# RuanJohn/Mava

Hardware: AMD Instinct MI355X
Metric: env-steps/sec (whole node), ff_mappo RWARE tiny-4ag (higher is better)
Workload: dtype f32 via 2 x f16 split operands on the MFMA (3 products, f32 accumulate); 1 GPU; ff_mappo RWARE tiny-4ag-shaped synthetic obs, 4096 envs/GPU (update_batch_size=1 x num_envs=4096), rollout_length=128, ppo_epochs=4, num_minibatches=2, agents=4, obs=70/264, actions=5, one step = one PPO update = 524288 env-steps per GPU; parallelism=dp1

## Files before the change

### include/mava_hip.h

```cpp
#ifndef MAVA_HIP_H
#define MAVA_HIP_H

#include <stddef.h>
#include <stdint.h>

#ifdef __cplusplus
extern "C" {
#endif

typedef struct ihipStream_t* mava_stream_t;

const char* mava_last_error(void);
int mava_abi_version(void);

typedef struct mava_ctx mava_ctx;
enum {
  MAVA_CTX_MATMUL_MODE = 0,
  MAVA_CTX_CRITIC_AGGREGATION = 1,
  MAVA_CTX_GAE_VARIANT = 2,
  MAVA_CTX_POLICY_VARIANT = 3,
  MAVA_CTX_H2_LAUNCHES = 4,
  MAVA_CTX_TRAIN_VARIANT = 5,
  MAVA_CTX_W8_LAUNCHES = 6,
  MAVA_CTX_W1_SPLIT_FRESH = 7
};
int mava_ctx_create(mava_ctx** out);
int mava_ctx_destroy(mava_ctx* ctx);
int mava_ctx_set(mava_ctx* ctx, int key, long value);
int mava_ctx_get(const mava_ctx* ctx, int key, long* value);

int mava_gae_f32(const mava_ctx* ctx, const float* reward, const float* value, const uint8_t* done,
                 const float* last_val, const uint8_t* last_done, int T, int N, float gamma,
                 float lambda, float* adv, float* tgt, mava_stream_t s);

int mava_permutation_i32(long n, uint64_t seed, uint64_t counter, int32_t* out, mava_stream_t s);

int mava_clip_adam(float* p, const float* g, float* m, float* v, int32_t* count,
                   const int* seg_off, const float* seg_lr, int n_seg, float grad_scale,
                   float max_norm, int decay, int steps_per_update, int num_updates, float b1,
                   float b2, float eps, const float* loss_sums, float vf_coef, float ent_coef,
                   float* metrics_out, mava_stream_t s);

size_t mava_ppo_finish_workspace_bytes(int Pa, int Pc);
int mava_ppo_finish_f32(mava_ctx* ctx, const float* slab_a, long stride_a, const float* slab_c, long stride_c, int n_slab,
                        int Pa, int Pc, float* g, float* p, float* m, float* v, int32_t* count, float lr_a, float lr_c,
                        float grad_scale, float max_norm, int decay, int steps_per_update, int num_updates, float b1,
                        float b2, float eps, float vf_coef, float ent_coef, float* metrics_out, int critic_din,
                        void* workspace, size_t workspace_bytes, mava_stream_t s);

int mava_slab_reduce_f32(const float* slab, int n_slab, long slab_stride, int n, int accumulate,
                         float* out, mava_stream_t s);

int mava_slab_reduce2_f32(const float* slab, int n_slab, long slab_stride, int n_main,
                          float* out_main, int n_tail, float* out_tail, int accumulate,
                          mava_stream_t s);

int mava_mlp_param_count(int din, int n_out);
// ... 345 lines not shown
```

### mava_amd/_lib.py

```python
from __future__ import annotations

import ctypes as C
import os
from typing import Optional

import torch

_HERE = os.path.dirname(os.path.abspath(__file__))
LIB_PATH = os.environ.get("MAVA_LIB_PATH") or os.path.join(_HERE, "libmavahip.so")

_lib: Optional[C.CDLL] = None


class MavaHipError(RuntimeError):
    pass


vp = C.c_void_p
i32 = C.c_int
u32 = C.c_uint32
u64 = C.c_uint64
f32 = C.c_float
lng = C.c_long

# ... 92 lines not shown
    "mava_mat_gelu_bwd_f32": [vp, vp, lng, vp, vp],
    "mava_mat_shift_onehot_f32": [vp, vp, i32, i32, i32, i32, lng, i32, vp, vp],
    "mava_mat_sample_f32": [i32, i32, i32, i32, vp, vp, u64, u32, u32, i32, vp, vp, vp],
    "mava_mat_loss_f32": [i32, i32, i32, lng, vp, vp, vp, vp, vp, vp, vp, vp, vp, vp, i32, f32, f32, f32, f32, vp, vp, vp, i32, vp],
}
_RESTYPES = {"mava_last_error": C.c_char_p, "mava_rec_step_pack_bytes": C.c_long, "mava_ppo_finish_workspace_bytes": C.c_size_t}


def declared_symbols():
    return sorted(set(_SIGNATURES) | set(_RESTYPES))


def lib() -> C.CDLL:
    global _lib
    if _lib is None:
        if not os.path.exists(LIB_PATH):
            raise MavaHipError(
                f"{LIB_PATH} is missing: build it with `python -m mava_amd.build` "
                "(hipcc --offload-arch=gfx950). There is no CPU fallback."
            )
        _lib = C.CDLL(LIB_PATH)
        _lib.mava_last_error.restype = C.c_char_p
        _lib.mava_last_error.argtypes = []
        for name, args in _SIGNATURES.items():
            fn = getattr(_lib, name)
            fn.argtypes = args
            fn.restype = _RESTYPES.get(name, C.c_int)
    return _lib


class Ctx:

    MATMUL_MODE, CRITIC_AGGREGATION, GAE_VARIANT, POLICY_VARIANT, H2_LAUNCHES, TRAIN_VARIANT, W8_LAUNCHES, W1_SPLIT_FRESH = 0, 1, 2, 3, 4, 5, 6, 7

    def __init__(self, matmul_mode: str = "f32", critic_aggregation: bool = True):
        if matmul_mode not in ("f32", "f16x2"):
            raise ValueError(f"matmul_mode must be 'f16x2' or 'f32', got {matmul_mode!r}")
        h = C.c_void_p()
        check(lib().mava_ctx_create(C.byref(h)), "mava_ctx_create")
        self.handle: Optional[int] = h.value
        self.set(self.MATMUL_MODE, 1 if matmul_mode == "f16x2" else 0)
        self.set(self.CRITIC_AGGREGATION, int(bool(critic_aggregation)))

    def set(self, key: int, value: int) -> None:
        check(lib().mava_ctx_set(self.handle, key, int(value)), "mava_ctx_set")

    def get(self, key: int) -> int:
        out = C.c_long()
        check(lib().mava_ctx_get(self.handle, key, C.byref(out)), "mava_ctx_get")
        return int(out.value)

    @property
    def matmul_mode(self) -> str:
        return "f16x2" if self.get(self.MATMUL_MODE) == 1 else "f32"

    @property
    def h2_launches(self) -> int:
        return self.get(self.H2_LAUNCHES)

    def close(self) -> None:
        if getattr(self, "handle", None) is not None and _lib is not None:
            _lib.mava_ctx_destroy(self.handle)
        self.handle = None

    def __del__(self):
        try:
# ... 41 lines not shown
```

### mava_amd/csrc/api.cpp

```cpp
#include <stdarg.h>
#include <stdio.h>
#include <string.h>

#include "common.h"
#include "ctx.h"

static thread_local char g_err[512] = "";

void mava_set_error(const char* fmt, ...) {
  va_list ap;
  va_start(ap, fmt);
  vsnprintf(g_err, sizeof(g_err), fmt, ap);
  va_end(ap);
}

extern "C" const char* mava_last_error(void) { return g_err; }

extern "C" int mava_abi_version(void) { return 3; }

enum { CTX_MATMUL_MODE = 0, CTX_CRITIC_AGGREGATION = 1, CTX_GAE_VARIANT = 2, CTX_POLICY_VARIANT = 3, CTX_H2_LAUNCHES = 4, CTX_TRAIN_VARIANT = 5, CTX_W8_LAUNCHES = 6, CTX_W1_SPLIT_FRESH = 7 };

extern "C" int mava_ctx_create(mava_ctx** out) {
  MAVA_ARG_CHECK(out != nullptr, 0, "mava_ctx_create: null output pointer");
  mava_ctx* c = new mava_ctx();
  c->matmul_mode = 0;
  c->critic_aggregation = 1;
  c->gae_variant = 0;
  c->policy_variant = 0;
  c->h2_launches = 0;
  c->train_variant = 0;
  c->w8_launches = 0;
  c->w1_split[0] = c->w1_split[1] = nullptr;
  for (int i = 0; i < 2; ++i) {
    c->w1_fresh[i] = 0;
    c->w1_key_params[i] = nullptr;
    c->w1_key_din[i] = c->w1_key_steps[i] = 0;
  }
  *out = c;
  return MAVA_OK;
}

extern "C" int mava_ctx_destroy(mava_ctx* c) {
  if (c == nullptr) return MAVA_OK;
  for (int i = 0; i < 2; ++i)
    if (c->w1_split[i] != nullptr) (void)hipFree(c->w1_split[i]);
  delete c;
  return MAVA_OK;
}

extern "C" int mava_ctx_set(mava_ctx* c, int key, long value) {
  MAVA_ARG_CHECK(c != nullptr, 0, "mava_ctx_set: null context");
  switch (key) {
    case CTX_MATMUL_MODE:
      MAVA_ARG_CHECK(value == 0 || value == 1, 1, "mava_ctx_set: matmul mode %ld (0 = exact f32, 1 = f16x2)", value);
      c->matmul_mode = (int)value;
      c->w1_fresh[0] = c->w1_fresh[1] = 0;
      return MAVA_OK;
    case CTX_CRITIC_AGGREGATION: c->critic_aggregation = value ? 1 : 0; return MAVA_OK;
    case CTX_GAE_VARIANT: c->gae_variant = (int)value; return MAVA_OK;
    case CTX_POLICY_VARIANT: c->policy_variant = (int)value; return MAVA_OK;
    case CTX_H2_LAUNCHES: c->h2_launches = value; return MAVA_OK;
    case CTX_TRAIN_VARIANT: c->train_variant = (int)value; return MAVA_OK;
    case CTX_W8_LAUNCHES: c->w8_launches = value; return MAVA_OK;
    case CTX_W1_SPLIT_FRESH:
      MAVA_ARG_CHECK(value == 0, 1, "mava_ctx_set: MAVA_CTX_W1_SPLIT_FRESH can only be cleared (0) by the caller");
      c->w1_fresh[0] = c->w1_fresh[1] = 0;
      return MAVA_OK;
    default: mava_set_error("mava_ctx_set: unknown key %d", key); return MAVA_EARG(2);
  }
}

extern "C" int mava_ctx_get(const mava_ctx* c, int key, long* value) {
  MAVA_ARG_CHECK(c != nullptr && value != nullptr, 0, "mava_ctx_get: null argument");
  switch (key) {
    case CTX_MATMUL_MODE: *value = c->matmul_mode; return MAVA_OK;
    case CTX_CRITIC_AGGREGATION: *value = c->critic_aggregation; return MAVA_OK;
    case CTX_GAE_VARIANT: *value = c->gae_variant; return MAVA_OK;
    case CTX_POLICY_VARIANT: *value = c->policy_variant; return MAVA_OK;
    case CTX_H2_LAUNCHES: *value = c->h2_launches; return MAVA_OK;
    case CTX_TRAIN_VARIANT: *value = c->train_variant; return MAVA_OK;
    case CTX_W8_LAUNCHES: *value = c->w8_launches; return MAVA_OK;
    case CTX_W1_SPLIT_FRESH: *value = c->w1_fresh[1]; return MAVA_OK;
    default: mava_set_error("mava_ctx_get: unknown key %d", key); return MAVA_EARG(2);
  }
}
```

### mava_amd/csrc/ctx.h

```cpp
#pragma once
#include "common.h"

struct mava_ctx {
  int matmul_mode;
  int critic_aggregation;
  int gae_variant;
  int policy_variant;
  int train_variant;
  long h2_launches;
  long w8_launches;
  void* w1_split[2];
  int w1_fresh[2];
  const float* w1_key_params[2];
  int w1_key_din[2];
  int w1_key_steps[2];
};

static inline int mava_ctx_matmul_mode(const mava_ctx* c) { return c ? c->matmul_mode : 0; }
static inline int mava_ctx_critic_aggregation(const mava_ctx* c) { return c ? c->critic_aggregation : 1; }
static inline int mava_ctx_gae_variant(const mava_ctx* c) { return c ? c->gae_variant : 0; }
static inline int mava_ctx_policy_variant(const mava_ctx* c) { return c ? c->policy_variant : 0; }
```

### mava_amd/csrc/ppo_train_h2.hip

```cpp
#include "h2_core.h"
#include "ppo_train_task.h"
#include "ctx.h"

#ifndef MAVA_GW_DEPTH
#define MAVA_GW_DEPTH 0
#endif
#define GW_DEPTH MAVA_GW_DEPTH
#ifndef MAVA_GW_DEPTH_WIDE
#define MAVA_GW_DEPTH_WIDE 0
#endif

namespace {

using namespace h2;

constexpr int STATS_BLOCKS = 128;

#ifdef MAVA_STAMPS
#define STAMP_DECL unsigned long long st_prev = __builtin_readcyclecounter(), st_acc[16] = {0, 0, 0, 0, 0, 0, 0, 0, 0, 0, 0, 0, 0, 0, 0, 0};
#define STAMP(i)                                                    \
  do {                                                              \
    __builtin_amdgcn_sched_barrier(0);                              \
    const unsigned long long st_now = __builtin_readcyclecounter(); \
    st_acc[i] += st_now - st_prev;                                  \
    st_prev = st_now;                                               \
    __builtin_amdgcn_sched_barrier(0);                              \
  } while (0)
#else
#define STAMP_DECL
#define STAMP(i)
#endif

struct H2Layout {
  int h1, dz2, dz1, w2, xs, xs_plane, xs_row, dy, yp, agg, small, end;
};
// ... 27 lines not shown

template <int NO, int S1, bool ACTOR, bool WIDE, int XV, int ROLE>
__device__ __forceinline__ void h2_body(const TrainTask& tk, const H2Layout& L, const uint4* __restrict__ w1p, u8* lds) {
  static_assert(!WIDE || S1 % W1_RING == 0, "WIDE: S1 must be a multiple of the W1 ring depth");
  static_assert((ROLE == 0) == !WIDE, "roles 1 / 2 belong to WIDE launches");
  constexpr bool CHAIN = ROLE != 2, LOADER = ROLE != 1;
#if defined(MAVA_NO_W2_RESIDENT) || defined(MAVA_W2_RESIDENT_P4)
  constexpr bool W2_RESIDENT = false;
#else
  constexpr bool W2_RESIDENT = !WIDE && NO <= 16;
#endif
#ifdef MAVA_W2_RESIDENT_P4
  constexpr bool W2_RES4 = !WIDE && ACTOR && NO <= 16;
#else
  constexpr bool W2_RES4 = false;
#endif
  constexpr int NTHR = WIDE ? 512 : 256;
  constexpr float WS = ACTOR ? 1.0f : W_SCALE_CRITIC, WU = 1.0f / WS;
  constexpr int KT1 = (S1 + 1) / 2;
  u8* const H1I = lds + L.h1;
  u8* const DZ2I = lds + L.dz2;
  u8* const DZ1I = lds + L.dz1;
  u8* const H2I = lds + L.dz1;
  u8* const W2I = lds + L.w2;
  u8* const DYI = lds + L.dy;
  float* const YP = reinterpret_cast<float*>(lds + L.yp);
  float* const AGG = reinterpret_cast<float*>(lds + L.agg);
  float* const B2s = reinterpret_cast<float*>(lds + L.small);
  float* const B3s = B2s + 128;
  float* const misc = B3s + 32;
  float* const W3s = misc + 16;
  const int xs_row = L.xs_row, xs_plane = L.xs_plane;

  const int tid = threadIdx.x & 255;
  const int lane = tid & 63, w = tid >> 6, h = lane >> 5, r = lane & 31;
  const int srow = tid >> 3, l8 = tid & 7;
  const int din = tk.din, no = tk.no;
  const long R = (!ACTOR && tk.agg > 1) ? (long)tk.Rb : (long)tk.Rb * tk.A;
  const float invR = 1.0f / (float)((long)tk.Rb * tk.A);
  constexpr int NPC = (32 * KT1 / XV + 7) / 8;
  constexpr int NR = NPC * XV;

  for (int i = threadIdx.x * 16; i < L.end; i += NTHR * 16) *reinterpret_cast<uint4*>(lds + i) = make_uint4(0, 0, 0, 0);
  __syncthreads();
  const float* const P = tk.params;
  const int oW2 = mlp_off_w2(din), oW3 = mlp_off_w3(din);
  if (CHAIN) {
    if (tid < 128) B2s[tid] = P[mlp_off_b2(din) + tid];
    if (tid < no) B3s[tid] = P[mlp_off_b3(din, no) + tid];
    if (!ACTOR && tid < 128) W3s[tid] = P[oW3 + tid];
    if (tid < (WIDE ? 32 : 64)) {
      const int b = tid >> 5, row = tid & 31;
      *reinterpret_cast<_Float16*>(lds + L.xs + b * 2 * xs_plane + row * xs_row + 2 * din) = (_Float16)1.0f;
    }
    {
      const int n = tid & 127, k0 = 64 * (tid >> 7);
      float carry = 0.0f;
#pragma unroll 8
      for (int k = k0; k < k0 + 64; ++k) {
        _Float16 x0, x1;
        split1_carry(P[oW2 + k * MLP_H + n] * WS, carry, x0, x1);
        const int o = sw_off(k, n >> 3) + 2 * (n & 7);
        *reinterpret_cast<_Float16*>(W2I + o) = x0;
        *reinterpret_cast<_Float16*>(W2I + W2_PLANE + o) = x1;
      }
    }
    if (ACTOR && tid == 0) {
      double s1 = 0.0, s2 = 0.0;
      for (int i = 0; i < STATS_BLOCKS; ++i) { s1 += tk.stats[2 * i]; s2 += tk.stats[2 * i + 1]; }
      const double mean = s1 / (double)R;
      double var = s2 / (double)R - mean * mean;
      if (var < 0.0) var = 0.0;
      misc[0] = (float)mean;
      misc[1] = 1.0f / ((float)sqrt(var) + 1e-8f);
    }
  }
  constexpr int S_LO = (WIDE && !CHAIN) ? S1 / 2 : 0, S_HI = (WIDE && CHAIN) ? S1 / 2 : S1, RL = S_HI - S_LO;
  static_assert(!WIDE || ((S1 / 2) % W1_RING == 0 && (S1 - S1 / 2) % W1_RING == 0), "WIDE: both halves must be multiples of the ring");
  constexpr int NW1 = WIDE ? W1_RING : (CHAIN ? S1 : 1);
  Frag W1f[NW1];
  const uint4* w1p_lane = w1p + 2 * (w * 64 + lane);
  auto w1_fetch = [&](int s) -> Frag {
    Frag f;
    f.hi = __builtin_bit_cast(half8, w1p_lane[512 * s]);
    f.lo = __builtin_bit_cast(half8, w1p_lane[512 * s + 1]);
    return f;
  };
  float w1_carry = 0.0f;
#pragma unroll
  for (int s = 0; s < (CHAIN ? NW1 : 0); ++s) {
    if (WIDE) {
      W1f[s] = w1_fetch(S_LO + s);
    } else {
      float v[8];
#pragma unroll
      for (int e = 0; e < 8; ++e) {
        const int k = 16 * s + 8 * h + e;
        v[e] = (k <= din) ? P[k * MLP_H + 32 * w + r] * WS : 0.0f;
      }
      W1f[s] = split8_carry(v, w1_carry);
    }
  }
  Frag W3h[2];
#pragma unroll
  for (int s = 0; s < ((CHAIN && ACTOR) ? 2 : 0); ++s) {
    float v[8];
#pragma unroll
    for (int e = 0; e < 8; ++e) {
      const int f = 32 * w + 16 * s + 8 * (e >> 2) + 4 * h + (e & 3);
      v[e] = (r < no) ? P[oW3 + f * no + r] * W3_SCALE : 0.0f;
    }
    W3h[s] = split8(v);
  }
  constexpr int ND = NO > 16 ? 2 : 1;
  Frag W3d[ND];
  if (CHAIN && ACTOR) {
#pragma unroll
    for (int s = 0; s < ND; ++s) {
// ... 66 lines not shown
    if (c.a >= Au) { c.a -= Au; c.b += 1u; }
  };
  auto cursor_gather = [&](const Cursor& c, int32_t& p_raw, uint32_t& a_out) {
    const bool in = c.q < (uint32_t)R;
    const uint32_t b = in ? c.b : b_last;
    a_out = in ? c.a : a_last;
    p_raw = tk.idx ? tk.idx[b] : (int32_t)(tk.idx_base + (long)b);
  };
  auto stage_row = [&](int32_t p_raw, uint32_t a) -> uint32_t {
    const uint32_t fr = (uint32_t)p_raw * Au + a;
    return (tk.xshare == 1) ? fr : ((uint32_t)tk.xshare == Au ? (uint32_t)p_raw : fr / (uint32_t)tk.xshare);
  };
  const int nv = din / XV;
  auto stage_issue = [&](uint32_t xrow_idx, float (&xr)[NR]) {
    const float* xrow = tk.x + (long)xrow_idx * din;
#pragma unroll
    for (int i = 0; i < NPC; ++i) {
      const int c = l8 + 8 * i;
      const int cc = (c < nv) ? c : 0;
      if (XV == 4) {
        const float4 v = reinterpret_cast<const float4*>(xrow)[cc];
        xr[4 * i] = v.x; xr[4 * i + 1] = v.y; xr[4 * i + 2] = v.z; xr[4 * i + 3] = v.w;
      } else if (XV == 2) {
        const float2 v = reinterpret_cast<const float2*>(xrow)[cc];
        xr[2 * i] = v.x; xr[2 * i + 1] = v.y;
      } else {
        xr[i] = xrow[cc];
      }
    }
  };
  u8* const xs_dummy = reinterpret_cast<u8*>(misc + 8);
  unsigned* const xflag = reinterpret_cast<unsigned*>(misc + 2);
  int tpar = 0;
  auto stage_commit = [&](int buf, const float (&xr)[NR], int flag_slot = 0) {
    u8* base = lds + L.xs + buf * 2 * xs_plane + srow * xs_row;
    uint32_t lo_any = 0;
#pragma unroll
    for (int i = 0; i < NPC; ++i) {
      const int c = l8 + 8 * i;
      const bool ok = c < nv;
      u8* qa = ok ? (base + 2 * XV * c) : xs_dummy;
      u8* qb = ok ? (base + xs_plane + 2 * XV * c) : xs_dummy;
      if (XV == 4) {
        half4 a, b;
#pragma unroll
        for (int e = 0; e < 4; ++e) { _Float16 x0, x1; split1(xr[4 * i + e], x0, x1); a[e] = x0; b[e] = x1; }
        *reinterpret_cast<half4*>(qa) = a;
        *reinterpret_cast<half4*>(qb) = b;
        if constexpr (WIDE) {
          const uint2 bb = __builtin_bit_cast(uint2, b);
          lo_any |= (bb.x | bb.y) & 0x7FFF7FFFu;
        }
      } else if (XV == 2) {
        typedef _Float16 half2v __attribute__((ext_vector_type(2)));
        half2v a, b;
#pragma unroll
        for (int e = 0; e < 2; ++e) { _Float16 x0, x1; split1(xr[2 * i + e], x0, x1); a[e] = x0; b[e] = x1; }
        *reinterpret_cast<half2v*>(qa) = a;
        *reinterpret_cast<half2v*>(qb) = b;
        if constexpr (WIDE) lo_any |= __builtin_bit_cast(uint32_t, b) & 0x7FFF7FFFu;
      } else {
        _Float16 x0, x1;
        split1(xr[i], x0, x1);
        *reinterpret_cast<_Float16*>(qa) = x0;
        *reinterpret_cast<_Float16*>(qb) = x1;
        if constexpr (WIDE) lo_any |= (uint32_t)__builtin_bit_cast(uint16_t, x1) & 0x7FFFu;
      }
    }
    if constexpr (WIDE) {
      if (lo_any != 0) xflag[flag_slot] = 1u;
    }
  };

  const long ntiles = (R + 31) / 32;
  long it = blockIdx.x;
  float xr[NR];
  int r_act[NP] = {}, n_act[NP] = {};
  float r_f0[NP] = {}, r_f1[NP] = {}, n_f0[NP] = {}, n_f1[NP] = {};
  uint32_t r_m[NP] = {}, n_m[NP] = {};
  Cursor cs = cursor_at(srow), cl[NP];
#pragma unroll
  for (int q = 0; q < NP; ++q) cl[q] = cursor_at(loss_row(q));
  int32_t ps_next = 0, pl_next[NP] = {};
  uint32_t as_next = 0, al_next[NP] = {};
  if (it < ntiles) {
    if (LOADER) {
      cursor_gather(cs, ps_next, as_next);
      stage_issue(stage_row(ps_next, as_next), xr);
    }
    if (CHAIN) {
#pragma unroll
      for (int q = 0; q < NP; ++q) {
        cursor_gather(cl[q], pl_next[q], al_next[q]);
        load_row((long)((uint32_t)pl_next[q] * Au + al_next[q]), r_act[q], r_f0[q], r_f1[q], r_m[q]);
      }
    }
    if (LOADER) {
      stage_commit(0, xr);
      cursor_advance(cs);
    }
    if (CHAIN) {
#pragma unroll
      for (int q = 0; q < NP; ++q) cursor_advance(cl[q]);
    }
    if (it + gridDim.x < ntiles) {
      if (LOADER) {
        cursor_gather(cs, ps_next, as_next);
        cursor_advance(cs);
      }
      if (CHAIN) {
#pragma unroll
        for (int q = 0; q < NP; ++q) cursor_gather(cl[q], pl_next[q], al_next[q]);
#pragma unroll
        for (int q = 0; q < NP; ++q) cursor_advance(cl[q]);
      }
    }
  }
  __syncthreads();

  const SwRow rowB = sw_row(r, h);
  const SwTr trS = sw_tr(lane);
  const int i16 = lane & 15, tq = i16 >> 2, tp = i16 & 3, g1 = (lane >> 4) & 1;
  const int trX = (8 * h + tq) * xs_row + 2 * (16 * g1 + 4 * tp);
  const int trD = (8 * h + tq) * DY_ROW + 2 * (16 * g1 + 4 * tp);
  const SwRow w2row = sw_row(32 * w + r, h);
  int buf = 0;
  Frag w2r[(W2_RESIDENT || W2_RES4) ? 8 : 1];
  if constexpr (W2_RESIDENT) {
#pragma unroll
    for (int s = 0; s < 8; ++s) w2r[s] = sw_read_tr(W2I, W2_PLANE, trS, s, w);
  }
  if constexpr (W2_RES4) {
#pragma unroll
    for (int s = 0; s < 8; ++s) w2r[s] = sw_read_row(W2I, W2_PLANE, w2row, s);
  }

  STAMP_DECL
  for (; it < ntiles; it += gridDim.x, buf ^= (WIDE ? 0 : 1), tpar ^= 1) {
    STAMP(14);
    const bool valid = (it * 32 + r) < R;
    const long itn = it + gridDim.x;
    const bool have_next = itn < ntiles;
    uint32_t xrow_next = LOADER ? stage_row(ps_next, as_next) : 0u;
    uint32_t fr_next[NP];
#pragma unroll
    for (int q = 0; q < NP; ++q) fr_next[q] = CHAIN ? ((uint32_t)pl_next[q] * Au + al_next[q]) : 0u;
    if (LOADER) asm volatile("" : "+v"(xrow_next));
    if (CHAIN) {
#pragma unroll
      for (int q = 0; q < NP; ++q) asm volatile("" : "+v"(fr_next[q]));
    }
    const u8* const XSI = lds + L.xs + buf * 2 * xs_plane;

    f32x16 acc;
    uint32_t relu1 = 0;
    if constexpr (WIDE) asm volatile("" : "+v"(w1p_lane));
    if constexpr (CHAIN || WIDE) {
#pragma unroll
    for (int q = 0; q < 16; ++q) acc[q] = 0.0f;
    if constexpr (WIDE && !CHAIN) {
#pragma unroll
      for (int s = 0; s < NW1; ++s) W1f[s] = w1_fetch(S_LO + s);
    }
    Frag xb = read_row_frag(XSI, xs_plane, r * xs_row + 16 * h + 32 * S_LO);
#pragma unroll
    for (int j = 0; j < RL; ++j) {
      const Frag b = xb;
      if (j + 1 < RL) xb = read_row_frag(XSI, xs_plane, r * xs_row + 16 * h + 32 * (S_LO + j + 1));
      acc = mfma3(W1f[j % NW1], b, acc);
      if (WIDE) {
        if (j >= 1 && j - 1 + W1_RING < RL) W1f[(j - 1) % NW1] = w1_fetch(S_LO + j - 1 + W1_RING);
      }
      __builtin_amdgcn_sched_barrier(0);
    }
    }
    if constexpr (WIDE) {
      float4* const xch = reinterpret_cast<float4*>(DZ2I) + (w * 4) * 64 + lane;
      if constexpr (LOADER) {
#pragma unroll
        for (int g = 0; g < 4; ++g) xch[g * 64] = make_float4(acc[4 * g], acc[4 * g + 1], acc[4 * g + 2], acc[4 * g + 3]);
      }
      __syncthreads();
      if constexpr (CHAIN) {
#pragma unroll
        for (int g = 0; g < 4; ++g) {
          const float4 v = xch[g * 64];
          acc[4 * g] += v.x; acc[4 * g + 1] += v.y; acc[4 * g + 2] += v.z; acc[4 * g + 3] += v.w;
        }
      }
    }
    if constexpr (CHAIN) {
    STAMP(0);
#pragma unroll
    for (int q = 0; q < 16; ++q) {
      acc[q] = fmaxf(ACTOR ? acc[q] : acc[q] * WU, 0.0f);
      relu1 |= (acc[q] > 0.0f) ? (1u << q) : 0u;
    }
    {
      half4 ph[4], pl[4];
      sw_write_image(H1I, r, w, h, acc, ph, pl);
    }
    }
    STAMP(1);
    if constexpr (WIDE && LOADER) {
      stage_issue(have_next ? xrow_next : 0u, xr);
    }
    if constexpr (WIDE && CHAIN) {
#pragma unroll
      for (int q = 0; q < NP; ++q) {
        asm volatile("" : "+v"(fr_next[q]));
        asm volatile("" : "+v"(cl[q].q), "+v"(cl[q].b), "+v"(cl[q].a));
      }
      asm volatile("" : "+v"(slot_c));
    }
    if (have_next) {
      if (LOADER && !WIDE) stage_issue(xrow_next, xr);
      const bool more = itn + gridDim.x < ntiles;
      if (more) {
        if (LOADER) {
          cursor_gather(cs, ps_next, as_next);
          cursor_advance(cs);
        }
        if (CHAIN) {
          Cursor c_old[NP];
#pragma unroll
          for (int q = 0; q < NP; ++q) { c_old[q] = cl[q]; cursor_advance(cl[q]); }
          __builtin_amdgcn_sched_barrier(0);
#pragma unroll
          for (int q = 0; q < NP; ++q) cursor_gather(c_old[q], pl_next[q], al_next[q]);
        }
      }
      if (CHAIN) {
#pragma unroll
        for (int q = 0; q < NP; ++q) load_row((long)fr_next[q], n_act[q], n_f0[q], n_f1[q], n_m[q]);
      }
    }
    if constexpr (WIDE && CHAIN) {
      __builtin_amdgcn_sched_barrier(0);
#pragma unroll
      for (int s2 = 0; s2 < NW1; ++s2) W1f[s2] = w1_fetch(S_LO + s2);
      __builtin_amdgcn_sched_barrier(0);
    }
    STAMP(2);
    __syncthreads();
    STAMP(3);

    f32x16 h2;
    uint32_t relu2 = 0;
// ... 29 lines not shown
#pragma unroll
      for (int q = 0; q < 16; ++q) {
        const float4 t = w3g[q >> 2];
        const float w3 = (q & 3) == 0 ? t.x : (q & 3) == 1 ? t.y : (q & 3) == 2 ? t.z : t.w;
        part = fmaf(h2[q], w3, part);
      }
      part += __shfl_xor(part, 32, 64);
      if (h == 0) YP[(w * 32 + r) * (NO + 1)] = part;
    } else {
      half4 ph[4], pl[4];
      sw_write_image(H2I, r, w, h, h2, ph, pl);
      f32x16 yacc;
#pragma unroll
      for (int q = 0; q < 16; ++q) yacc[q] = 0.0f;
#pragma unroll
      for (int s = 0; s < 2; ++s) {
        Frag b;
        b.hi = __builtin_shufflevector(ph[2 * s], ph[2 * s + 1], 0, 1, 2, 3, 4, 5, 6, 7);
        b.lo = __builtin_shufflevector(pl[2 * s], pl[2 * s + 1], 0, 1, 2, 3, 4, 5, 6, 7);
        yacc = mfma3(W3h[s], b, yacc);
      }
#pragma unroll
      for (int q = 0; q < 16; ++q) {
        const int o = (q & 3) + 8 * (q >> 2) + 4 * h;
        if ((q & 3) + 8 * (q >> 2) < NO) {
          if (o < NO) YP[(w * 32 + r) * (NO + 1) + o] = yacc[q] * W3_UNSCALE;
        }
      }
    }
    }
    STAMP(5);
    __syncthreads();
    STAMP(6);

    f32x16 dz;
    float dy0 = 0.0f;
    if constexpr (CHAIN) {
    if (ACTOR) {
      const float lo_c = 1.0f - tk.clip_eps, hi_c = 1.0f + tk.clip_eps;
#pragma unroll
      for (int q = 0; q < NP; ++q) {
        const int row = loss_row(q);
        const bool rvalid = (it * 32 + row) < R;
        const float* yp = YP + row * (NO + 1) + lo;
        const float y = (((yp[0] + yp[32 * (NO + 1)]) + yp[2 * 32 * (NO + 1)]) + yp[3 * 32 * (NO + 1)]) + B3s[lo];
        const bool legal = (lo < no) && (r_m[q] != 0u);
        const float z = legal ? y : -FLT_MAX;
        auto fmax_op = [](float a, float b) { return fmaxf(a, b); };
        auto add_op = [](float a, float b) { return a + b; };
        const float mx = group_allreduce<NO>(z, fmax_op);
        const float se = group_allreduce<NO>(expf(z - mx), add_op);
        const float logp = (mx == -FLT_MAX) ? ((lo < no) ? -logf((float)no) : -FLT_MAX) : z - (mx + logf(se));
        const float pr = expf(logp);
        const float ent = group_allreduce<NO>((pr > 0.0f) ? -(pr * logp) : 0.0f, add_op);
        const int act = r_act[q];
        const float lp = group_allreduce<NO>((lo == act) ? logp : 0.0f, add_op);
        const float gae = (r_f1[q] - adv_mean) * adv_rstd;
        const float ratio = expf(lp - r_f0[q]);
        const float rc = fminf(fmaxf(ratio, lo_c), hi_c);
        const float l1 = ratio * gae, l2 = rc * gae;
        const float pg = -fminf(l1, l2);
        const bool inside = (ratio >= lo_c) && (ratio <= hi_c);
        const float g1 = (l1 < l2) ? 1.0f : ((l1 == l2) ? 0.5f : 0.0f);
        const float g2 = inside ? (1.0f - g1) : 0.0f;
        const float dlp = rvalid ? (-(g1 + g2) * gae * ratio) : 0.0f;
        const float ec = rvalid ? tk.ent_coef : 0.0f;
// ... 111 lines not shown
        for (int s = 0; s < 2; ++s) {
          const Frag b = sw_read_tr(DZ2I, SW_PLANE, trS, s, w);
#pragma unroll
          for (int t = 0; t < 4; ++t) {
            const Frag a = sw_read_tr(H1I, SW_PLANE, trS, s, t);
            gW2[t] = mfma3(a, b, gW2[t]);
            if (t & 1) __builtin_amdgcn_sched_barrier(0);
          }
        }
      }
    };
    if constexpr (CHAIN) {
#pragma unroll
      for (int q = 0; q < 16; ++q) acc[q] = 0.0f;
      Frag an;
      if constexpr (!W2_RES4) an = sw_read_row(W2I, W2_PLANE, w2row, 0);
      Frag bn = sw_read_row(DZ2I, SW_PLANE, rowB, 0);
#pragma unroll
      for (int s = 0; s < 8; ++s) {
        const Frag a = W2_RES4 ? w2r[s] : an, b = bn;
        if (s + 1 < 8) {
          if constexpr (!W2_RES4) an = sw_read_row(W2I, W2_PLANE, w2row, s + 1);
          bn = sw_read_row(DZ2I, SW_PLANE, rowB, s + 1);
        }
        acc = mfma3(a, b, acc);
        __builtin_amdgcn_sched_barrier(0);
      }
#pragma unroll
      for (int q = 0; q < 16; ++q) acc[q] = ((relu1 >> q) & 1u) ? (ACTOR ? acc[q] : acc[q] * WU) : 0.0f;
      half4 ph[4], pl[4];
      sw_write_image(DZ1I, r, w, h, acc, ph, pl);
    }
    if constexpr (!WIDE) {
      if (have_next) stage_commit(buf ^ 1, xr);
    }
    STAMP(10);
    if constexpr (!WIDE) do_gw2();
    STAMP(11);
    __syncthreads();
    STAMP(12);
    if constexpr (WIDE && CHAIN) do_gw2();
    bool x_lo = true;
    if constexpr (WIDE && LOADER) {
      x_lo = __builtin_amdgcn_readfirstlane((int)xflag[tpar]) != 0 || tk.force_xlo != 0;
      if (tid == 0) xflag[tpar ^ 1] = 0u;
    }
    if constexpr (LOADER) {
      constexpr int NPR = 2 * KT1;
      constexpr int D1 = WIDE ? MAVA_GW_DEPTH_WIDE : GW_DEPTH;
      if (WIDE && D1 > 0 && !x_lo) {
        constexpr int DP = (D1 > 0 ? (D1 < NPR ? D1 : NPR) : 1);
        const Frag b0 = sw_read_tr(DZ1I, SW_PLANE, trS, 0, w), b1 = sw_read_tr(DZ1I, SW_PLANE, trS, 1, w);
        half8 a[DP];
#pragma unroll
        for (int i = 0; i < DP; ++i) a[i] = read_tr8(XSI + trX + 16 * (i / KT1) * xs_row + 2 * (32 * (i % KT1)), xs_row);
#pragma unroll
        for (int i = 0; i < NPR; ++i) {
          const half8 cur = a[i % DP];
          if (i + DP < NPR) a[i % DP] = read_tr8(XSI + trX + 16 * ((i + DP) / KT1) * xs_row + 2 * (32 * ((i + DP) % KT1)), xs_row);
          const Frag& b = (i / KT1) ? b1 : b0;
          f32x16 c = gW1[i % KT1];
          c = __builtin_amdgcn_mfma_f32_32x32x16_f16(cur, b.lo, c, 0, 0, 0);
          gW1[i % KT1] = __builtin_amdgcn_mfma_f32_32x32x16_f16(cur, b.hi, c, 0, 0, 0);
          __builtin_amdgcn_sched_barrier(0);
        }
      } else if constexpr (D1 > 0) {
        constexpr int DP = D1 < NPR ? D1 : NPR;
        const Frag b0 = sw_read_tr(DZ1I, SW_PLANE, trS, 0, w), b1 = sw_read_tr(DZ1I, SW_PLANE, trS, 1, w);
        Frag a[DP > 0 ? DP : 1];
#pragma unroll
        for (int i = 0; i < DP; ++i) a[i] = read_tr_frag(XSI + trX + 16 * (i / KT1) * xs_row + 2 * (32 * (i % KT1)), xs_plane, xs_row);
#pragma unroll
        for (int i = 0; i < NPR; ++i) {
          const Frag cur = a[i % (DP > 0 ? DP : 1)];
          if (i + DP < NPR)
            a[i % (DP > 0 ? DP : 1)] = read_tr_frag(XSI + trX + 16 * ((i + DP) / KT1) * xs_row + 2 * (32 * ((i + DP) % KT1)), xs_plane, xs_row);
          gW1[i % KT1] = mfma3(cur, (i / KT1) ? b1 : b0, gW1[i % KT1]);
          __builtin_amdgcn_sched_barrier(0);
        }
      } else {
#pragma unroll
        for (int s = 0; s < 2; ++s) {
          const Frag b = sw_read_tr(DZ1I, SW_PLANE, trS, s, w);
#pragma unroll
          for (int t = 0; t < KT1; ++t) {
            const Frag a = read_tr_frag(XSI + trX + 16 * s * xs_row + 2 * (32 * t), xs_plane, xs_row);
            gW1[t] = mfma3(a, b, gW1[t]);
            if (t & 1) __builtin_amdgcn_sched_barrier(0);
          }
        }
      }
    }
    STAMP(13);
    if constexpr (WIDE) {
      __syncthreads();
      if constexpr (LOADER) {
        stage_commit(0, xr, tpar ^ 1);
      }
      __syncthreads();
    }
    if constexpr (CHAIN) {
#pragma unroll
      for (int q = 0; q < NP; ++q) { r_act[q] = n_act[q]; r_f0[q] = n_f0[q]; r_f1[q] = n_f1[q]; r_m[q] = n_m[q]; }
    }
  }
#ifdef MAVA_STAMPS
  if (tk.stamps != nullptr && blockIdx.x == 0 && lane == 0) {
    for (int i = 0; i < 16; ++i) tk.stamps[((ROLE == 2 ? 4 : 0) + w) * 16 + i] = st_acc[i];
  }
#endif

  __syncthreads();
  float* slab = tk.slab + (long)blockIdx.x * tk.slab_stride;
  const int oB2 = mlp_off_b2(din), oB3 = mlp_off_b3(din, no);
  const int Pn = mlp_param_count(din, no);
  if constexpr (LOADER) {
#pragma unroll
    for (int t = 0; t < KT1; ++t)
#pragma unroll
      for (int q = 0; q < 16; ++q) {
        const int k = mlp_feat(t, q, h);
        if (k <= din) slab[k * MLP_H + 32 * w + r] = gW1[t][q] * invR;
      }
  }
  if constexpr (CHAIN) {
#pragma unroll
    for (int t = 0; t < 4; ++t)
#pragma unroll
      for (int q = 0; q < 16; ++q) slab[oW2 + mlp_feat(t, q, h) * MLP_H + 32 * w + r] = gW2[t][q] * invR;
#pragma unroll
    for (int q = 0; q < 16; ++q) {
      float v = ab2[q];
#pragma unroll
      for (int m = 1; m < 32; m <<= 1) v += __shfl_xor(v, m, 64);
      if (r == 0) slab[oB2 + 32 * w + (q & 3) + 8 * (q >> 2) + 4 * h] = v * invR;
    }
  }
  float* red = reinterpret_cast<float*>(lds + L.h1);
  if constexpr (!CHAIN) {
    __syncthreads();
  } else if (ACTOR) {
#pragma unroll
    for (int q = 0; q < 16; ++q) {
      const int o = (q & 3) + 8 * (q >> 2) + 4 * h;
      if (o < no) slab[oW3 + (32 * w + r) * no + o] = gW3[q] * invR;
// ... 45 lines not shown
      h2_body<NO, S1, ACTOR, WIDE, XV, 1>(tk, L, w1p, lds);
    } else {
      h2_body<NO, S1, ACTOR, WIDE, XV, 2>(tk, L, w1p, lds);
    }
  } else {
    h2_body<NO, S1, ACTOR, WIDE, XV, 0>(tk, L, w1p, lds);
  }
}

template <int NO, int S1, bool ACTOR, bool WIDE, int XV>
int launch_h2(mava_ctx* ctx, const TrainTask& tk, int n_slab, hipStream_t s) {
  const H2Layout L = make_h2_layout<NO, S1, WIDE>(ACTOR);
  MAVA_ARG_CHECK(L.end <= 163840, 8, "ppo_train_h2: %d bytes of LDS exceed the 160 KiB of a CU", L.end);
  static bool attr_set = false;
  if (!attr_set) {
    MAVA_HIP_CHECK(hipFuncSetAttribute((const void*)ppo_train_h2_kernel<NO, S1, ACTOR, WIDE, XV>,
                                       hipFuncAttributeMaxDynamicSharedMemorySize, L.end));
    attr_set = true;
  }
  const uint4* w1p = nullptr;
  if (WIDE) {
    void*& slot = ctx->w1_split[ACTOR ? 0 : 1];
    if (slot == nullptr) MAVA_HIP_CHECK(hipMalloc(&slot, W1_SPLIT_BYTES));
    uint4* const buf = static_cast<uint4*>(slot);
    const int kind = ACTOR ? 0 : 1;
    int& fresh = ctx->w1_fresh[kind];
    const bool keyed = ctx->w1_key_params[kind] == tk.params && ctx->w1_key_din[kind] == tk.din && ctx->w1_key_steps[kind] == S1;
    if (!(fresh && keyed)) {
      hipLaunchKernelGGL((pack_w1_kernel<S1>), dim3(1), dim3(256), 0, s, tk.params, tk.din, buf, ACTOR ? 1.0f : W_SCALE_CRITIC);
      MAVA_LAUNCH_CHECK();
    }
    fresh = 0;
    w1p = buf;
  }
  g_train_last_instance = train_instance_id(2, ACTOR, false, WIDE, NO, S1, XV);
  hipLaunchKernelGGL((ppo_train_h2_kernel<NO, S1, ACTOR, WIDE, XV>), dim3(n_slab), dim3(WIDE ? 512 : 256), L.end, s, tk, L,
                     w1p);
  MAVA_LAUNCH_CHECK();
  return MAVA_OK;
}

template <int NO, int S1, bool ACTOR, bool WIDE>
int dispatch_xv(mava_ctx* ctx, const TrainTask& tk, int n_slab, hipStream_t s) {
  const uintptr_t a = (uintptr_t)tk.x;
  if constexpr (WIDE) {
    if (tk.din % 4 == 0 && a % 16 == 0) return launch_h2<NO, S1, ACTOR, WIDE, 4>(ctx, tk, n_slab, s);
  } else {
    if (tk.din % 2 == 0 && a % 8 == 0) return launch_h2<NO, S1, ACTOR, WIDE, 2>(ctx, tk, n_slab, s);
  }
  return launch_h2<NO, S1, ACTOR, WIDE, 1>(ctx, tk, n_slab, s);
}

template <int NO, bool ACTOR>
int dispatch_s1(mava_ctx* ctx, const TrainTask& tk, int n_slab, hipStream_t s) {
  const int s1 = (tk.din + 1 + 15) / 16;
  switch (s1) {
#ifndef MAVA_FAST_BUILD
    case 1: return dispatch_xv<NO, 1, ACTOR, false>(ctx, tk, n_slab, s);
    case 2: return dispatch_xv<NO, 2, ACTOR, false>(ctx, tk, n_slab, s);
    case 3: return dispatch_xv<NO, 3, ACTOR, false>(ctx, tk, n_slab, s);
    case 4: return dispatch_xv<NO, 4, ACTOR, false>(ctx, tk, n_slab, s);
    case 6: return dispatch_xv<NO, 6, ACTOR, false>(ctx, tk, n_slab, s);
    case 7: case 8: case 9: case 10: case 11: case 12: return dispatch_xv<NO, 12, ACTOR, true>(ctx, tk, n_slab, s);
#endif
    case 5: return dispatch_xv<NO, 5, ACTOR, false>(ctx, tk, n_slab, s);
    case 13: case 14: case 15: case 16: case 17: case 18: return dispatch_xv<NO, 18, ACTOR, true>(ctx, tk, n_slab, s);
    default: return 1;
  }
}
// ... 32 lines not shown
```

### mava_amd/csrc/ppo_train_task.h

```cpp
#pragma once
#include <stdint.h>

#include "common.h"

struct TrainTask {
  const float* params;
  const float* x;
  int din, no, xshare, xv;
  int A;
  int agg;
  const int32_t* idx;
  long idx_base;
  int Rb;
  const uint8_t* mask;
  const int32_t* action;
  const float* action_f;
  uint32_t seed_lo, seed_hi, ent_step, row_offset;
  float min_scale;
  const float* old_logp;
  const float* adv;
  const double* stats;
  const float* old_value;
  const float* targets;
  float clip_eps, ent_coef, vf_coef;
  float* slab;
  long slab_stride;
  unsigned long long* stamps;
  int force_xlo;
};

struct mava_ctx;
int mava_train_w8_launch(const TrainTask& tk, int n_slab, bool actor, hipStream_t s);
int mava_train_h2_launch(mava_ctx* ctx, const TrainTask& tk, int n_slab, bool actor, hipStream_t s);

extern int g_train_last_instance;
constexpr int train_instance_id(int family, bool actor, bool cont, bool wide, int no, int k, int xv) {
  return family * 1000000 + ((actor ? 1 : 0) + (cont ? 2 : 0) + (wide ? 4 : 0)) * 100000 + no * 1000 + k * 10 + xv;
}
```

Baseline: 75.07 million env-steps/s.

## Add exact-input loop version for wide critic that skips low-half f16 products

The wide critic training kernel now checks per tile whether the staged input's low f16 residual plane is all zero. While that holds, it runs a specialised loop body that stores only the high plane, uses two MFMA products instead of three in the forward pass, and uses a simpler weight-gradient path. When a nonzero low half shows up, it falls back to the general loop. A device counter of exact tiles is added to the context, and the next-row load/cursor schedule in the wide chain path is reworked. This adds code size and register pressure, plus a per-tile flag check and an atomic.

After: 78.28 million env-steps/s (median of 6 runs). 1.04x the previous value.

```diff
diff --git a/include/mava_hip.h b/include/mava_hip.h
--- a/include/mava_hip.h
+++ b/include/mava_hip.h
@@ -22,7 +22,8 @@
   MAVA_CTX_H2_LAUNCHES = 4,
   MAVA_CTX_TRAIN_VARIANT = 5,
   MAVA_CTX_W8_LAUNCHES = 6,
-  MAVA_CTX_W1_SPLIT_FRESH = 7
+  MAVA_CTX_W1_SPLIT_FRESH = 7,
+  MAVA_CTX_EXACT_TILES = 8
 };
 int mava_ctx_create(mava_ctx** out);
 int mava_ctx_destroy(mava_ctx* ctx);
diff --git a/mava_amd/_lib.py b/mava_amd/_lib.py
--- a/mava_amd/_lib.py
+++ b/mava_amd/_lib.py
@@ -148,6 +148,7 @@
 class Ctx:
 
     MATMUL_MODE, CRITIC_AGGREGATION, GAE_VARIANT, POLICY_VARIANT, H2_LAUNCHES, TRAIN_VARIANT, W8_LAUNCHES, W1_SPLIT_FRESH = 0, 1, 2, 3, 4, 5, 6, 7
+    EXACT_TILES = 8
 
     def __init__(self, matmul_mode: str = "f32", critic_aggregation: bool = True):
         if matmul_mode not in ("f32", "f16x2"):
diff --git a/mava_amd/csrc/api.cpp b/mava_amd/csrc/api.cpp
--- a/mava_amd/csrc/api.cpp
+++ b/mava_amd/csrc/api.cpp
@@ -18,7 +18,7 @@
 
 extern "C" int mava_abi_version(void) { return 3; }
 
-enum { CTX_MATMUL_MODE = 0, CTX_CRITIC_AGGREGATION = 1, CTX_GAE_VARIANT = 2, CTX_POLICY_VARIANT = 3, CTX_H2_LAUNCHES = 4, CTX_TRAIN_VARIANT = 5, CTX_W8_LAUNCHES = 6, CTX_W1_SPLIT_FRESH = 7 };
+enum { CTX_MATMUL_MODE = 0, CTX_CRITIC_AGGREGATION = 1, CTX_GAE_VARIANT = 2, CTX_POLICY_VARIANT = 3, CTX_H2_LAUNCHES = 4, CTX_TRAIN_VARIANT = 5, CTX_W8_LAUNCHES = 6, CTX_W1_SPLIT_FRESH = 7, CTX_EXACT_TILES = 8 };
 
 extern "C" int mava_ctx_create(mava_ctx** out) {
   MAVA_ARG_CHECK(out != nullptr, 0, "mava_ctx_create: null output pointer");
@@ -36,6 +36,7 @@
     c->w1_key_params[i] = nullptr;
     c->w1_key_din[i] = c->w1_key_steps[i] = 0;
   }
+  c->exact_tiles = nullptr;
   *out = c;
   return MAVA_OK;
 }
@@ -44,6 +45,7 @@
   if (c == nullptr) return MAVA_OK;
   for (int i = 0; i < 2; ++i)
     if (c->w1_split[i] != nullptr) (void)hipFree(c->w1_split[i]);
+  if (c->exact_tiles != nullptr) (void)hipFree(c->exact_tiles);
   delete c;
   return MAVA_OK;
 }
@@ -66,6 +68,13 @@
       MAVA_ARG_CHECK(value == 0, 1, "mava_ctx_set: MAVA_CTX_W1_SPLIT_FRESH can only be cleared (0) by the caller");
       c->w1_fresh[0] = c->w1_fresh[1] = 0;
       return MAVA_OK;
+    case CTX_EXACT_TILES:
+      MAVA_ARG_CHECK(value == 0, 1, "mava_ctx_set: MAVA_CTX_EXACT_TILES can only be reset (0) by the caller");
+      if (c->exact_tiles != nullptr) {
+        MAVA_HIP_CHECK(hipDeviceSynchronize());
+        MAVA_HIP_CHECK(hipMemset(c->exact_tiles, 0, sizeof(unsigned long long)));
+      }
+      return MAVA_OK;
     default: mava_set_error("mava_ctx_set: unknown key %d", key); return MAVA_EARG(2);
   }
 }
@@ -81,6 +90,15 @@
     case CTX_TRAIN_VARIANT: *value = c->train_variant; return MAVA_OK;
     case CTX_W8_LAUNCHES: *value = c->w8_launches; return MAVA_OK;
     case CTX_W1_SPLIT_FRESH: *value = c->w1_fresh[1]; return MAVA_OK;
+    case CTX_EXACT_TILES: {
+      unsigned long long n = 0;
+      if (c->exact_tiles != nullptr) {
+        MAVA_HIP_CHECK(hipDeviceSynchronize());
+        MAVA_HIP_CHECK(hipMemcpy(&n, c->exact_tiles, sizeof(n), hipMemcpyDeviceToHost));
+      }
+      *value = (long)n;
+      return MAVA_OK;
+    }
     default: mava_set_error("mava_ctx_get: unknown key %d", key); return MAVA_EARG(2);
   }
 }
diff --git a/mava_amd/csrc/ctx.h b/mava_amd/csrc/ctx.h
--- a/mava_amd/csrc/ctx.h
+++ b/mava_amd/csrc/ctx.h
@@ -14,6 +14,7 @@
   const float* w1_key_params[2];
   int w1_key_din[2];
   int w1_key_steps[2];
+  unsigned long long* exact_tiles;
 };
 
 static inline int mava_ctx_matmul_mode(const mava_ctx* c) { return c ? c->matmul_mode : 0; }
diff --git a/mava_amd/csrc/ppo_train_h2.hip b/mava_amd/csrc/ppo_train_h2.hip
--- a/mava_amd/csrc/ppo_train_h2.hip
+++ b/mava_amd/csrc/ppo_train_h2.hip
@@ -1,6 +1,8 @@
 #include "h2_core.h"
 #include "ppo_train_task.h"
 #include "ctx.h"
+
+#include <type_traits>
 
 #ifndef MAVA_GW_DEPTH
 #define MAVA_GW_DEPTH 0
@@ -94,9 +96,9 @@
   float* const W3s = misc + 16;
   const int xs_row = L.xs_row, xs_plane = L.xs_plane;
 
-  const int tid = threadIdx.x & 255;
-  const int lane = tid & 63, w = tid >> 6, h = lane >> 5, r = lane & 31;
-  const int srow = tid >> 3, l8 = tid & 7;
+  int tid = threadIdx.x & 255;
+  int lane = tid & 63, w = tid >> 6, h = lane >> 5, r = lane & 31;
+  int srow = tid >> 3, l8 = tid & 7;
   const int din = tk.din, no = tk.no;
   const long R = (!ACTOR && tk.agg > 1) ? (long)tk.Rb : (long)tk.Rb * tk.A;
   const float invR = 1.0f / (float)((long)tk.Rb * tk.A);
@@ -142,10 +144,13 @@
   constexpr int NW1 = WIDE ? W1_RING : (CHAIN ? S1 : 1);
   Frag W1f[NW1];
   const uint4* w1p_lane = w1p + 2 * (w * 64 + lane);
+  typedef unsigned u32x4 __attribute__((ext_vector_type(4)));
+  typedef const __attribute__((address_space(1))) u32x4* w1_gptr;
   auto w1_fetch = [&](int s) -> Frag {
+    const w1_gptr g = (w1_gptr)w1p_lane;
     Frag f;
-    f.hi = __builtin_bit_cast(half8, w1p_lane[512 * s]);
-    f.lo = __builtin_bit_cast(half8, w1p_lane[512 * s + 1]);
+    f.hi = __builtin_bit_cast(half8, g[512 * s]);
+    f.lo = __builtin_bit_cast(half8, g[512 * s + 1]);
     return f;
   };
   float w1_carry = 0.0f;
@@ -278,8 +283,9 @@
   u8* const xs_dummy = reinterpret_cast<u8*>(misc + 8);
   unsigned* const xflag = reinterpret_cast<unsigned*>(misc + 2);
   int tpar = 0;
-  auto stage_commit = [&](int buf, const float (&xr)[NR], int flag_slot = 0) {
-    u8* base = lds + L.xs + buf * 2 * xs_plane + srow * xs_row;
+  auto stage_commit = [&](auto hi_only_tag, auto flag_tag, u8* dst, const float (&xr)[NR], int flag_slot) {
+    constexpr bool HI_ONLY = decltype(hi_only_tag)::value, FLAG = decltype(flag_tag)::value;
+    u8* base = dst + srow * xs_row;
     uint32_t lo_any = 0;
 #pragma unroll
     for (int i = 0; i < NPC; ++i) {
@@ -292,8 +298,8 @@
 #pragma unroll
         for (int e = 0; e < 4; ++e) { _Float16 x0, x1; split1(xr[4 * i + e], x0, x1); a[e] = x0; b[e] = x1; }
         *reinterpret_cast<half4*>(qa) = a;
-        *reinterpret_cast<half4*>(qb) = b;
-        if constexpr (WIDE) {
+        if constexpr (!HI_ONLY) *reinterpret_cast<half4*>(qb) = b;
+        if constexpr (FLAG) {
           const uint2 bb = __builtin_bit_cast(uint2, b);
           lo_any |= (bb.x | bb.y) & 0x7FFF7FFFu;
         }
@@ -303,20 +309,24 @@
 #pragma unroll
         for (int e = 0; e < 2; ++e) { _Float16 x0, x1; split1(xr[2 * i + e], x0, x1); a[e] = x0; b[e] = x1; }
         *reinterpret_cast<half2v*>(qa) = a;
-        *reinterpret_cast<half2v*>(qb) = b;
-        if constexpr (WIDE) lo_any |= __builtin_bit_cast(uint32_t, b) & 0x7FFF7FFFu;
+        if constexpr (!HI_ONLY) *reinterpret_cast<half2v*>(qb) = b;
+        if constexpr (FLAG) lo_any |= __builtin_bit_cast(uint32_t, b) & 0x7FFF7FFFu;
       } else {
         _Float16 x0, x1;
         split1(xr[i], x0, x1);
         *reinterpret_cast<_Float16*>(qa) = x0;
-        *reinterpret_cast<_Float16*>(qb) = x1;
-        if constexpr (WIDE) lo_any |= (uint32_t)__builtin_bit_cast(uint16_t, x1) & 0x7FFFu;
-      }
-    }
-    if constexpr (WIDE) {
+        if constexpr (!HI_ONLY) *reinterpret_cast<_Float16*>(qb) = x1;
+        if constexpr (FLAG) lo_any |= (uint32_t)__builtin_bit_cast(uint16_t, x1) & 0x7FFFu;
+      }
+    }
+    if constexpr (FLAG) {
       if (lo_any != 0) xflag[flag_slot] = 1u;
     }
   };
+  using std::false_type;
+  using std::true_type;
+  constexpr bool VERSIONED = WIDE && !ACTOR;
+  using versioned_tag = std::bool_constant<VERSIONED>;
 
   const long ntiles = (R + 31) / 32;
   long it = blockIdx.x;
@@ -342,7 +352,7 @@
       }
     }
     if (LOADER) {
-      stage_commit(0, xr);
+      stage_commit(false_type{}, versioned_tag{}, lds + L.xs, xr, 0);
       cursor_advance(cs);
     }
     if (CHAIN) {
@@ -364,12 +374,12 @@
   }
   __syncthreads();
 
-  const SwRow rowB = sw_row(r, h);
-  const SwTr trS = sw_tr(lane);
+  SwRow rowB = sw_row(r, h);
+  SwTr trS = sw_tr(lane);
   const int i16 = lane & 15, tq = i16 >> 2, tp = i16 & 3, g1 = (lane >> 4) & 1;
-  const int trX = (8 * h + tq) * xs_row + 2 * (16 * g1 + 4 * tp);
+  int trX = (8 * h + tq) * xs_row + 2 * (16 * g1 + 4 * tp);
   const int trD = (8 * h + tq) * DY_ROW + 2 * (16 * g1 + 4 * tp);
-  const SwRow w2row = sw_row(32 * w + r, h);
+  SwRow w2row = sw_row(32 * w + r, h);
   int buf = 0;
   Frag w2r[(W2_RESIDENT || W2_RES4) ? 8 : 1];
   if constexpr (W2_RESIDENT) {
@@ -382,11 +392,18 @@
   }
 
   STAMP_DECL
-  for (; it < ntiles; it += gridDim.x, buf ^= (WIDE ? 0 : 1), tpar ^= 1) {
+  bool exact = false;
+  unsigned n_exact = 0;
+  auto tile_body = [&](auto exact_tag) __attribute__((always_inline)) {
+    constexpr bool EXACT = decltype(exact_tag)::value;
+    static_assert(!EXACT || VERSIONED, "the exact-input loop belongs to the wide critic");
     STAMP(14);
     const bool valid = (it * 32 + r) < R;
     const long itn = it + gridDim.x;
     const bool have_next = itn < ntiles;
+    if constexpr (EXACT && LOADER) {
+      if (tid == 0) xflag[tpar ^ 1] = 0u;
+    }
     uint32_t xrow_next = LOADER ? stage_row(ps_next, as_next) : 0u;
     uint32_t fr_next[NP];
 #pragma unroll
@@ -396,7 +413,7 @@
 #pragma unroll
       for (int q = 0; q < NP; ++q) asm volatile("" : "+v"(fr_next[q]));
     }
-    const u8* const XSI = lds + L.xs + buf * 2 * xs_plane;
+    const u8* const XSI = lds + L.xs + (EXACT ? tpar : 2 * buf) * xs_plane;
 
     f32x16 acc;
     uint32_t relu1 = 0;
@@ -408,12 +425,22 @@
 #pragma unroll
       for (int s = 0; s < NW1; ++s) W1f[s] = w1_fetch(S_LO + s);
     }
-    Frag xb = read_row_frag(XSI, xs_plane, r * xs_row + 16 * h + 32 * S_LO);
+    Frag xb;
+    xb.hi = *reinterpret_cast<const half8*>(XSI + r * xs_row + 16 * h + 32 * S_LO);
+    if constexpr (!EXACT) xb.lo = *reinterpret_cast<const half8*>(XSI + xs_plane + r * xs_row + 16 * h + 32 * S_LO);
 #pragma unroll
     for (int j = 0; j < RL; ++j) {
       const Frag b = xb;
-      if (j + 1 < RL) xb = read_row_frag(XSI, xs_plane, r * xs_row + 16 * h + 32 * (S_LO + j + 1));
-      acc = mfma3(W1f[j % NW1], b, acc);
+      if (j + 1 < RL) {
+        xb.hi = *reinterpret_cast<const half8*>(XSI + r * xs_row + 16 * h + 32 * (S_LO + j + 1));
+        if constexpr (!EXACT) xb.lo = *reinterpret_cast<const half8*>(XSI + xs_plane + r * xs_row + 16 * h + 32 * (S_LO + j + 1));
+      }
+      if constexpr (EXACT) {
+        acc = __builtin_amdgcn_mfma_f32_32x32x16_f16(W1f[j % NW1].lo, b.hi, acc, 0, 0, 0);
+        acc = __builtin_amdgcn_mfma_f32_32x32x16_f16(W1f[j % NW1].hi, b.hi, acc, 0, 0, 0);
+      } else {
+        acc = mfma3(W1f[j % NW1], b, acc);
+      }
       if (WIDE) {
         if (j >= 1 && j - 1 + W1_RING < RL) W1f[(j - 1) % NW1] = w1_fetch(S_LO + j - 1 + W1_RING);
       }
@@ -459,7 +486,24 @@
       }
       asm volatile("" : "+v"(slot_c));
     }
-    if (have_next) {
+    if constexpr (WIDE && CHAIN) {
+      if (have_next) {
+        const bool more = itn + gridDim.x < ntiles;
+        Cursor c_old[NP];
+        if (more) {
+#pragma unroll
+          for (int q = 0; q < NP; ++q) { c_old[q] = cl[q]; cursor_advance(cl[q]); }
+        }
+        __builtin_amdgcn_sched_barrier(0);
+#pragma unroll
+        for (int q = 0; q < NP; ++q) load_row((long)fr_next[q], n_act[q], n_f0[q], n_f1[q], n_m[q]);
+        __builtin_amdgcn_sched_barrier(0);
+        if (more) {
+#pragma unroll
+          for (int q = 0; q < NP; ++q) cursor_gather(c_old[q], pl_next[q], al_next[q]);
+        }
+      }
+    } else if (have_next) {
       if (LOADER && !WIDE) stage_issue(xrow_next, xr);
       const bool more = itn + gridDim.x < ntiles;
       if (more) {
@@ -555,6 +599,9 @@
     STAMP(5);
     __syncthreads();
     STAMP(6);
+    if constexpr (EXACT && LOADER) {
+      stage_commit(true_type{}, true_type{}, lds + L.xs + (tpar ^ 1) * xs_plane, xr, tpar ^ 1);
+    }
 
     f32x16 dz;
     float dy0 = 0.0f;
@@ -732,7 +779,7 @@
       sw_write_image(DZ1I, r, w, h, acc, ph, pl);
     }
     if constexpr (!WIDE) {
-      if (have_next) stage_commit(buf ^ 1, xr);
+      if (have_next) stage_commit(false_type{}, false_type{}, lds + L.xs + (buf ^ 1) * 2 * xs_plane, xr, 0);
     }
     STAMP(10);
     if constexpr (!WIDE) do_gw2();
@@ -740,29 +787,20 @@
     __syncthreads();
     STAMP(12);
     if constexpr (WIDE && CHAIN) do_gw2();
-    bool x_lo = true;
-    if constexpr (WIDE && LOADER) {
-      x_lo = __builtin_amdgcn_readfirstlane((int)xflag[tpar]) != 0 || tk.force_xlo != 0;
-      if (tid == 0) xflag[tpar ^ 1] = 0u;
-    }
     if constexpr (LOADER) {
       constexpr int NPR = 2 * KT1;
       constexpr int D1 = WIDE ? MAVA_GW_DEPTH_WIDE : GW_DEPTH;
-      if (WIDE && D1 > 0 && !x_lo) {
-        constexpr int DP = (D1 > 0 ? (D1 < NPR ? D1 : NPR) : 1);
-        const Frag b0 = sw_read_tr(DZ1I, SW_PLANE, trS, 0, w), b1 = sw_read_tr(DZ1I, SW_PLANE, trS, 1, w);
-        half8 a[DP];
-#pragma unroll
-        for (int i = 0; i < DP; ++i) a[i] = read_tr8(XSI + trX + 16 * (i / KT1) * xs_row + 2 * (32 * (i % KT1)), xs_row);
-#pragma unroll
-        for (int i = 0; i < NPR; ++i) {
-          const half8 cur = a[i % DP];
-          if (i + DP < NPR) a[i % DP] = read_tr8(XSI + trX + 16 * ((i + DP) / KT1) * xs_row + 2 * (32 * ((i + DP) % KT1)), xs_row);
-          const Frag& b = (i / KT1) ? b1 : b0;
-          f32x16 c = gW1[i % KT1];
-          c = __builtin_amdgcn_mfma_f32_32x32x16_f16(cur, b.lo, c, 0, 0, 0);
-          gW1[i % KT1] = __builtin_amdgcn_mfma_f32_32x32x16_f16(cur, b.hi, c, 0, 0, 0);
-          __builtin_amdgcn_sched_barrier(0);
+      if constexpr (EXACT) {
+#pragma unroll
+        for (int s = 0; s < 2; ++s) {
+          const Frag b = sw_read_tr(DZ1I, SW_PLANE, trS, s, w);
+#pragma unroll
+          for (int t = 0; t < KT1; ++t) {
+            const half8 a = read_tr8(XSI + trX + 16 * s * xs_row + 2 * (32 * t), xs_row);
+            const f32x16 c = __builtin_amdgcn_mfma_f32_32x32x16_f16(a, b.lo, gW1[t], 0, 0, 0);
+            gW1[t] = __builtin_amdgcn_mfma_f32_32x32x16_f16(a, b.hi, c, 0, 0, 0);
+            if (t & 1) __builtin_amdgcn_sched_barrier(0);
+          }
         }
       } else if constexpr (D1 > 0) {
         constexpr int DP = D1 < NPR ? D1 : NPR;
@@ -794,16 +832,37 @@
     STAMP(13);
     if constexpr (WIDE) {
       __syncthreads();
-      if constexpr (LOADER) {
-        stage_commit(0, xr, tpar ^ 1);
-      }
+      if constexpr (EXACT) {
+        exact = __builtin_amdgcn_readfirstlane((int)xflag[tpar ^ 1]) == 0;
+        ++n_exact;
+      } else {
+        if constexpr (LOADER) {
+          stage_commit(false_type{}, false_type{}, lds + L.xs, xr, 0);
+        }
+        __syncthreads();
+      }
+    }
+    if constexpr (CHAIN) {
+#pragma unroll
+      for (int q = 0; q < NP; ++q) { r_act[q] = n_act[q]; r_f0[q] = n_f0[q]; r_f1[q] = n_f1[q]; r_m[q] = n_m[q]; }
+    }
+  };
+  if constexpr (VERSIONED) {
+    exact = __builtin_amdgcn_readfirstlane((int)xflag[0]) == 0 && tk.force_xlo == 0;
+    if (exact && it < ntiles) {
+      if (CHAIN && tid < 32) *reinterpret_cast<_Float16*>(lds + L.xs + xs_plane + tid * xs_row + 2 * din) = (_Float16)1.0f;
+    }
+    for (; it < ntiles && exact; it += gridDim.x, tpar ^= 1) tile_body(true_type{});
+    asm volatile("" : "+v"(tid), "+v"(lane), "+v"(w), "+v"(h), "+v"(r), "+v"(trS.b0), "+v"(trS.b1), "+v"(trS.q64));
+    if constexpr (LOADER) asm volatile("" : "+v"(srow), "+v"(l8), "+v"(trX));
+    if constexpr (CHAIN) asm volatile("" : "+v"(rowB.base), "+v"(rowB.hx), "+v"(w2row.base), "+v"(w2row.hx));
+    if (n_exact != 0 && it < ntiles) {
+      if constexpr (LOADER) stage_commit(false_type{}, false_type{}, lds + L.xs, xr, 0);
+      if (CHAIN && tid < 32) *reinterpret_cast<_Float16*>(lds + L.xs + xs_plane + tid * xs_row + 2 * din) = (_Float16)0.0f;
       __syncthreads();
     }
-    if constexpr (CHAIN) {
-#pragma unroll
-      for (int q = 0; q < NP; ++q) { r_act[q] = n_act[q]; r_f0[q] = n_f0[q]; r_f1[q] = n_f1[q]; r_m[q] = n_m[q]; }
-    }
-  }
+  }
+  for (; it < ntiles; it += gridDim.x, buf ^= (WIDE ? 0 : 1)) tile_body(false_type{});
 #ifdef MAVA_STAMPS
   if (tk.stamps != nullptr && blockIdx.x == 0 && lane == 0) {
     for (int i = 0; i < 16; ++i) tk.stamps[((ROLE == 2 ? 4 : 0) + w) * 16 + i] = st_acc[i];
@@ -811,6 +870,9 @@
 #endif
 
   __syncthreads();
+  if constexpr (VERSIONED && CHAIN) {
+    if (tid == 0 && tk.exact_tiles != nullptr) atomicAdd(tk.exact_tiles, (unsigned long long)n_exact);
+  }
   float* slab = tk.slab + (long)blockIdx.x * tk.slab_stride;
   const int oB2 = mlp_off_b2(din), oB3 = mlp_off_b3(din, no);
   const int Pn = mlp_param_count(din, no);
@@ -922,9 +984,17 @@
     }
     fresh = 0;
     w1p = buf;
-  }
+    if (ctx->exact_tiles == nullptr) {
+      void* word = nullptr;
+      MAVA_HIP_CHECK(hipMalloc(&word, sizeof(unsigned long long)));
+      ctx->exact_tiles = static_cast<unsigned long long*>(word);
+      MAVA_HIP_CHECK(hipMemsetAsync(word, 0, sizeof(unsigned long long), s));
+    }
+  }
+  TrainTask tkl = tk;
+  tkl.exact_tiles = WIDE ? ctx->exact_tiles : nullptr;
   g_train_last_instance = train_instance_id(2, ACTOR, false, WIDE, NO, S1, XV);
-  hipLaunchKernelGGL((ppo_train_h2_kernel<NO, S1, ACTOR, WIDE, XV>), dim3(n_slab), dim3(WIDE ? 512 : 256), L.end, s, tk, L,
+  hipLaunchKernelGGL((ppo_train_h2_kernel<NO, S1, ACTOR, WIDE, XV>), dim3(n_slab), dim3(WIDE ? 512 : 256), L.end, s, tkl, L,
                      w1p);
   MAVA_LAUNCH_CHECK();
   return MAVA_OK;
diff --git a/mava_amd/csrc/ppo_train_task.h b/mava_amd/csrc/ppo_train_task.h
--- a/mava_amd/csrc/ppo_train_task.h
+++ b/mava_amd/csrc/ppo_train_task.h
@@ -27,6 +27,7 @@
   long slab_stride;
   unsigned long long* stamps;
   int force_xlo;
+  unsigned long long* exact_tiles;
 };
 
 struct mava_ctx;
```
